# barrust/pyprobables

Measured on AMD Instinct MI355X. Metric: million keys/sec insert+lookup (Bloom m=2^28 k=7, CMS 2^20x5), higher is better.
Workload: dtype u64; 1 GPU; cfg2 Bloom m=2^28 k=7: per rank per step clear + insert 10M 16B keys + (merge) + check them; keys_per_rank=10000000, key_bytes=16, m_bits=268435456, k=7, parallelism=single GPU

## Files before the change

### pyprobables_amd/csrc/psk_part_bins.hpp

```cpp
#pragma once
#include "psk_partition.hpp"

namespace psk {

#ifndef PSK_BINS_NT
#define PSK_BINS_NT 768
#endif
constexpr int kBinThreads = PSK_BINS_NT;
constexpr int kBinMinWaves = kBinThreads <= 512 ? 4 : (kBinThreads <= 768 ? 6 : 8);
#ifndef PSK_BINS_KPT
#define PSK_BINS_KPT 2
#endif
constexpr int kBinKpt = PSK_BINS_KPT;
constexpr int kBinSlicesPerLane = 2;

template <class Pay>
struct pay_bins_ok { static constexpr bool value = false; };
template <>
struct pay_bins_ok<PayNone> { static constexpr bool value = true; };
template <>
struct pay_bins_ok<PayTileTag> { static constexpr bool value = true; };
template <>
struct pay_bins_ok<PayWeightSmall> { static constexpr bool value = true; };

constexpr uint32_t kBinHead = 2;
template <class Src, class IdxFn, class Pay, class Spill, int KT, int KPT>
__global__ __launch_bounds__(kBinThreads, kBinMinWaves) void k_part_bins(Src src, IdxFn idxfn, Pay pay, Spill spill, PartGeom g, uint32_t n, uint32_t cap,
                                                              uint32_t stride, uint32_t *segcnt, uint4 *buckets)
{
    constexpr int NT = kBinThreads;
    extern __shared__ __attribute__((aligned(16))) uint32_t smem[];
    char *lds = reinterpret_cast<char *>(smem);
    const uint32_t B = g.nbuckets;
    constexpr bool kExactK = KT != 8;
    const uint32_t k = kExactK ? (uint32_t)KT : g.k;
    const uint32_t mask = (1u << g.shift) - 1;
    const uint32_t tk = g.tile;
    const uint32_t ntiles = (n + tk - 1) / tk;
    const uint32_t last = n ? n - 1 : 0;
    const uint32_t stride4 = stride * 4u;
    const uint32_t lg_slices = 31u - (uint32_t)__builtin_clz(B);
    const uint32_t full4 = (cap + kBinHead) * 4u;
    constexpr uint32_t kCnt = 4;

    uint32_t L = 1;
    while (2 * L * B <= (uint32_t)NT) L *= 2;
    constexpr int kSlicesPerLane = kBinSlicesPerLane;
    const uint32_t sub = B <= (uint32_t)NT ? threadIdx.x % L : 0u;
    uint32_t myb[kSlicesPerLane], cur[kSlicesPerLane];
    uint4 *seg[kSlicesPerLane];
#pragma unroll
    for (int s = 0; s < kSlicesPerLane; ++s) {
        myb[s] = B <= (uint32_t)NT ? (s == 0 && threadIdx.x / L < B ? threadIdx.x / L : ~0u) : threadIdx.x + (uint32_t)s * NT;
        if (myb[s] >= B) myb[s] = ~0u;
        cur[s] = 0;
        seg[s] = buckets + (seg_index(g, 0, blockIdx.x) + (myb[s] == ~0u ? 0u : myb[s])) * g.segcap;
    }
    for (uint32_t b = threadIdx.x; b < B; b += NT) *reinterpret_cast<uint32_t *>(lds + b * stride4 + kCnt) = kBinHead * 4u;

    const uint32_t dbg = kBenchKnobs ? g.dbg : 0u;
    unsigned long long *t_acc = reinterpret_cast<unsigned long long *>(lds + (size_t)B * stride4 + 32);
    unsigned long long t_prev = 0;
    const bool t_lane = (dbg & 32) && (threadIdx.x == 0 || threadIdx.x == NT - 64);
    const uint32_t t_base = threadIdx.x == 0 ? 0u : 4u;
    if ((dbg & 32) && threadIdx.x < 8) t_acc[threadIdx.x] = 0;
#define PSK_BIN_TICK(ph)                                                 \
    if (t_lane) {                                                        \
        const unsigned long long t_now = __builtin_readcyclecounter();   \
        t_acc[t_base + (ph)] += t_now - t_prev;                          \
        t_prev = t_now;                                                  \
    }
    uint32_t fold = 0;
    constexpr bool WP = pay_weighted_plain<Pay>::value;
    typename Src::Key kcur[KPT];
    uint32_t wcur[WP ? KPT : 1];
    long long tally_s = 0;
    unsigned long long tally_a = 0;
    uint32_t tally_b = 0;
    {
        const uint32_t b0 = blockIdx.x * tk;
#pragma unroll
        for (int q = 0; q < KPT; ++q) {
            const uint32_t i = b0 + (uint32_t)q * NT + threadIdx.x;
            kcur[q] = src.load(i < last ? i : last);
            if constexpr (WP) wcur[q] = pay(i < last ? i : last, 0);
        }
    }
    lds_barrier();
    if (t_lane) t_prev = __builtin_readcyclecounter();

    uint32_t ordinal = ~0u;
    for (uint32_t tile = blockIdx.x; tile < ntiles; tile += gridDim.x) {
        ++ordinal;
        const uint32_t base = tile * tk;
        const uint32_t tile_end = base + tk < n ? base + tk : n;
        if constexpr (PSK_EXP_PRIO == 1) __builtin_amdgcn_s_setprio(0);
#pragma unroll
        for (int q = 0; q < KPT; ++q) {
            const uint32_t i = base + (uint32_t)q * NT + threadIdx.x;
            if ((uint32_t)q * NT < tk && i < tile_end) {
                uint32_t val[KT], bin[KT];
                uint32_t wfield = 0, wbig = 0, wq = 0;
                if constexpr (WP) {
                    wq = wcur[q];
                    if (pay.tally) {
                        const long long v = pay.weights_signed ? (long long)(int32_t)wq : (long long)wq;
                        tally_s += v;
                        tally_a += (unsigned long long)(v < 0 ? -v : v);
                        tally_b += (uint32_t)(wq >= (1u << kSmallWeightBits));
                    }
                    wbig = wq >= (1u << kSmallWeightBits) ? 1u : 0u;
                    wfield = wbig ? 0u : wq << 15;
                }
                if constexpr (IdxFn::lo32) {
                    uint32_t h[KT];
                    if (dbg & 4) {
#pragma unroll
                        for (int j = 0; j < KT; ++j) h[j] = (uint32_t)(((uint64_t)(i * 2654435761u + (uint32_t)j * 40503u) * 0x9E3779B97F4A7C15ULL) >> 13);
                    } else {
                        src.template hash32<KT>(kcur[q], i, 0u, h);
                    }
#pragma unroll
                    for (int j = 0; j < KT; ++j) {
                        if constexpr (std::is_same<IdxFn, IdxBloom<true>>::value || std::is_same<IdxFn, IdxBloomWide<true>>::value) {
                            val[j] = h[j] & mask;
                            bin[j] = __builtin_amdgcn_ubfe(h[j], g.shift, lg_slices);
                        } else {
                            const uint32_t x = idxfn.from32((uint32_t)j, h[j]);
                            val[j] = x & mask;
                            bin[j] = x >> g.shift;
                        }
                    }
                } else {
                    uint64_t h[KT];
                    src.template hash<KT>(kcur[q], i, 0u, h);
#pragma unroll
                    for (int j = 0; j < KT; ++j) {
                        const uint32_t x = idxfn((uint32_t)j, h[j]);
                        val[j] = x & mask;
                        bin[j] = x >> g.shift;
                    }
                }
                if (dbg & 2) {
#pragma unroll
                    for (int j = 0; j < KT; ++j) fold ^= val[j] + bin[j];
                    continue;
                }
                uint32_t at[KT], r4[KT], worst = 0;
#pragma unroll
                for (int j = 0; j < KT; ++j) {
                    r4[j] = 0;
                    if ((uint32_t)j < k) {
                        at[j] = __umul24(bin[j], stride4);
                        r4[j] = atomicAdd(reinterpret_cast<uint32_t *>(lds + at[j] + kCnt), 4u);
                    }
                }
#pragma unroll
                for (int j = 0; j < KT; ++j) {
                    if ((uint32_t)j < k) {
                        worst = r4[j] > worst ? r4[j] : worst;
                        *reinterpret_cast<uint32_t *>(lds + at[j] + (r4[j] < full4 ? r4[j] : full4)) = WP ? (val[j] | wfield) : val[j];
                    }
                }
                if constexpr (WP) {
                    if (wbig) {
#pragma unroll
                        for (int j = 0; j < KT; ++j)
                            if ((uint32_t)j < k) spill((bin[j] << g.shift) | val[j], wq);
                    }
                }
                if (worst >= full4) {
#pragma unroll
                    for (int j = 0; j < KT; ++j)
                        if ((uint32_t)j < k && r4[j] >= full4) {
                            if constexpr (pay_tile_tag<Pay>::value) spill((bin[j] << g.shift) | val[j], tile);
                            else if constexpr (WP) { if (!wbig) spill((bin[j] << g.shift) | val[j], wq); }
                            else spill((bin[j] << g.shift) | val[j], 0u);
                        }
                }
            }
        }
        {
            const uint32_t nb = (tile + gridDim.x) * tk;
#pragma unroll
            for (int q = 0; q < KPT; ++q) {
                const uint32_t i = nb + (uint32_t)q * NT + threadIdx.x;
                kcur[q] = src.load(i < last ? i : last);
                if constexpr (WP) wcur[q] = pay(i < last ? i : last, 0);
            }
        }
        if (dbg & 2) {
            if (fold == 0x12345u) segcnt[0] = fold;
            continue;
        }
        PSK_BIN_TICK(0);
        lds_barrier();
        PSK_BIN_TICK(1);
        if constexpr (PSK_EXP_PRIO == 1) __builtin_amdgcn_s_setprio(3);

        const uint32_t t0 = pay_tile_tag<Pay>::value ? (ordinal & 3u) << 2 : 0u, t1 = pay_tile_tag<Pay>::value ? ordinal & 12u : 0u;
#pragma unroll
        for (int s = 0; s < kSlicesPerLane; ++s) {
            const uint32_t b = myb[s];
            if (b == ~0u) continue;
            const char *bin = lds + b * stride4;
            const uint32_t c4 = *reinterpret_cast<const uint32_t *>(bin + kCnt);
            const uint32_t c = ((c4 < full4 ? c4 : full4) >> 2) - kBinHead;
            const uint32_t whole = c / 6u, rem = c - 6u * whole, ngroups = whole + (rem ? 1u : 0u);
            const uint2 *e = reinterpret_cast<const uint2 *>(bin + kBinHead * 4u);
            uint4 *out = seg[s] + cur[s];
            if (cur[s] + ngroups <= g.segcap) {
                const uint32_t hi0 = (3u | t0) << 28, hi1 = (3u | t1) << 28;
                for (uint32_t gq = sub; gq < whole; gq += L) {
                    const uint2 a0 = e[3 * gq], a1 = e[3 * gq + 1], a2 = e[3 * gq + 2];
                    uint4 o;
                    o.x = a0.x | (a0.y << 20);
                    o.y = (a0.y >> 12) | (a1.x << 8) | hi0;
                    o.z = a1.y | (a2.x << 20);
                    o.w = (a2.x >> 12) | (a2.y << 8) | hi1;
                    if (!(dbg & 1)) out[gq] = o;
                }
                if (rem && sub == (whole & (L - 1))) {
                    const uint2 a0 = e[3 * whole], a1 = e[3 * whole + 1], a2 = e[3 * whole + 2];
                    uint32_t f[6] = {a0.x, a0.y, a1.x, a1.y, a2.x, a2.y};
#pragma unroll
                    for (int x = 1; x < 6; ++x)
                        if ((uint32_t)x >= rem) f[x] = WP ? 0u : mask;
                    const uint32_t n0 = rem < 3u ? rem : 3u, n1 = rem - n0;
                    uint4 o;
                    o.x = f[0] | (f[1] << 20);
                    o.y = (f[1] >> 12) | (f[2] << 8) | ((n0 | t0) << 28);
                    o.z = f[3] | (f[4] << 20);
                    o.w = (f[4] >> 12) | (f[5] << 8) | ((n1 | t1) << 28);
                    if (!(dbg & 1)) out[whole] = o;
                }
            } else {
                for (uint32_t gq = sub; gq < ngroups; gq += L) {
                    const uint2 a0 = e[3 * gq], a1 = e[3 * gq + 1], a2 = e[3 * gq + 2];
                    uint32_t f[6] = {a0.x, a0.y, a1.x, a1.y, a2.x, a2.y};
                    const uint32_t left = c - 6u * gq, nv = left < 6u ? left : 6u;
#pragma unroll
                    for (int x = 1; x < 6; ++x)
                        if ((uint32_t)x >= nv) f[x] = WP ? 0u : mask;
                    const uint32_t n0 = nv < 3u ? nv : 3u, n1 = nv - n0;
                    if (cur[s] + gq < g.segcap) {
                        uint4 o;
                        o.x = f[0] | (f[1] << 20);
                        o.y = (f[1] >> 12) | (f[2] << 8) | ((n0 | t0) << 28);
                        o.z = f[3] | (f[4] << 20);
                        o.w = (f[4] >> 12) | (f[5] << 8) | ((n1 | t1) << 28);
                        out[gq] = o;
                    } else {
#pragma unroll
                        for (int x = 0; x < 6; ++x)
                            if ((uint32_t)x < nv) {
                                if constexpr (pay_tile_tag<Pay>::value) spill((b << g.shift) | f[x], tile);
                                else if constexpr (WP) spill((b << g.shift) | (f[x] & mask), f[x] >> 15);
                                else spill((b << g.shift) | f[x], 0u);
                            }
                    }
                }
            }
            cur[s] += ngroups;
        }
#pragma unroll
        for (int s = 0; s < kSlicesPerLane; ++s)
            if (myb[s] != ~0u && sub == 0) *reinterpret_cast<uint32_t *>(lds + myb[s] * stride4 + kCnt) = kBinHead * 4u;
#pragma unroll
        for (int q = 0; q < KPT; ++q) {
            Src::pin(kcur[q]);
            if constexpr (WP) asm volatile("" : "+v"(wcur[q]));
        }
        PSK_BIN_TICK(2);
        lds_barrier();
        PSK_BIN_TICK(3);
    }
    if (t_lane) {
        unsigned long long *prof = reinterpret_cast<unsigned long long *>(segcnt + (size_t)g.nbuckets * g.nwg);
        for (int ph = 0; ph < 4; ++ph) atomicAdd(prof + 1 + t_base + ph, t_acc[t_base + ph]);
        if (threadIdx.x == 0) atomicAdd(prof, 1ULL);
    }
#undef PSK_BIN_TICK
    if constexpr (WP) {
        if (pay.tally) {
            for (int o = 32; o > 0; o >>= 1) {
                tally_s += __shfl_down(tally_s, o);
                tally_a += __shfl_down(tally_a, o);
                tally_b += __shfl_down(tally_b, o);
            }
            unsigned long long *red = reinterpret_cast<unsigned long long *>(smem);
            if ((threadIdx.x & 63) == 0) {
                red[3 * (threadIdx.x >> 6)] = (unsigned long long)tally_s;
                red[3 * (threadIdx.x >> 6) + 1] = tally_a;
                red[3 * (threadIdx.x >> 6) + 2] = tally_b;
            }
            lds_barrier();
            if (threadIdx.x == 0) {
                unsigned long long ss = 0, aa = 0, bb = 0;
                for (int w = 0; w < NT / 64; ++w) { ss += red[3 * w]; aa += red[3 * w + 1]; bb += red[3 * w + 2]; }
                pay.tally[blockIdx.x] = make_ulonglong4(ss, aa, bb, 0ULL);
            }
        }
    }
#pragma unroll
    for (int s = 0; s < kSlicesPerLane; ++s)
        if (myb[s] != ~0u && sub == 0) segcnt[(uint64_t)myb[s] * g.nwg + blockIdx.x] = cur[s] < g.segcap ? cur[s] : g.segcap;
}

}
```

Before: 61580 Mkeys/s.

## Software-pipeline hashing of next tile's first key slot across bin write-out

Restructures the partition-bins kernel loop so the hash chain for slot 0 of the next tile is computed before the LDS barrier, while the current tile's bins are being written out. Key loads for the tile after that are issued as each slot is consumed, rather than all together at the end of the tile. The aim is to overlap ALU hashing and global loads with the LDS write-out phase and the barrier stalls. The cost is extra live registers for the precomputed hash values, so it is gated per template by a maximum KT, with the old loop kept as a fallback.

```diff
diff --git a/pyprobables_amd/csrc/psk_part_bins.hpp b/pyprobables_amd/csrc/psk_part_bins.hpp
--- a/pyprobables_amd/csrc/psk_part_bins.hpp
+++ b/pyprobables_amd/csrc/psk_part_bins.hpp
@@ -13,6 +13,16 @@
 #endif
 constexpr int kBinKpt = PSK_BINS_KPT;
 constexpr int kBinSlicesPerLane = 2;
+#ifndef PSK_BINS_PIPE
+#define PSK_BINS_PIPE 1
+#endif
+constexpr bool kBinPipe = PSK_BINS_PIPE != 0;
+template <class Src, class IdxFn, class Pay, int KT>
+struct bins_pipe {
+    static constexpr bool kWeighted = pay_weighted_plain<Pay>::value, kMulti = std::is_same<Src, KeysFixed16Multi>::value;
+    static constexpr int kMaxKt = IdxFn::lo32 ? (kWeighted ? 5 : (kMulti ? 7 : 8)) : (kWeighted ? 4 : 5);
+    static constexpr bool value = kBinPipe && KT <= kMaxKt;
+};
 
 template <class Pay>
 struct pay_bins_ok { static constexpr bool value = false; };
@@ -77,127 +87,93 @@
     long long tally_s = 0;
     unsigned long long tally_a = 0;
     uint32_t tally_b = 0;
-    {
-        const uint32_t b0 = blockIdx.x * tk;
-#pragma unroll
-        for (int q = 0; q < KPT; ++q) {
-            const uint32_t i = b0 + (uint32_t)q * NT + threadIdx.x;
-            kcur[q] = src.load(i < last ? i : last);
-            if constexpr (WP) wcur[q] = pay(i < last ? i : last, 0);
-        }
-    }
-    lds_barrier();
-    if (t_lane) t_prev = __builtin_readcyclecounter();
-
-    uint32_t ordinal = ~0u;
-    for (uint32_t tile = blockIdx.x; tile < ntiles; tile += gridDim.x) {
-        ++ordinal;
-        const uint32_t base = tile * tk;
-        const uint32_t tile_end = base + tk < n ? base + tk : n;
-        if constexpr (PSK_EXP_PRIO == 1) __builtin_amdgcn_s_setprio(0);
-#pragma unroll
-        for (int q = 0; q < KPT; ++q) {
-            const uint32_t i = base + (uint32_t)q * NT + threadIdx.x;
-            if ((uint32_t)q * NT < tk && i < tile_end) {
-                uint32_t val[KT], bin[KT];
-                uint32_t wfield = 0, wbig = 0, wq = 0;
-                if constexpr (WP) {
-                    wq = wcur[q];
-                    if (pay.tally) {
-                        const long long v = pay.weights_signed ? (long long)(int32_t)wq : (long long)wq;
-                        tally_s += v;
-                        tally_a += (unsigned long long)(v < 0 ? -v : v);
-                        tally_b += (uint32_t)(wq >= (1u << kSmallWeightBits));
-                    }
-                    wbig = wq >= (1u << kSmallWeightBits) ? 1u : 0u;
-                    wfield = wbig ? 0u : wq << 15;
-                }
-                if constexpr (IdxFn::lo32) {
-                    uint32_t h[KT];
-                    if (dbg & 4) {
-#pragma unroll
-                        for (int j = 0; j < KT; ++j) h[j] = (uint32_t)(((uint64_t)(i * 2654435761u + (uint32_t)j * 40503u) * 0x9E3779B97F4A7C15ULL) >> 13);
-                    } else {
-                        src.template hash32<KT>(kcur[q], i, 0u, h);
-                    }
-#pragma unroll
-                    for (int j = 0; j < KT; ++j) {
-                        if constexpr (std::is_same<IdxFn, IdxBloom<true>>::value || std::is_same<IdxFn, IdxBloomWide<true>>::value) {
-                            val[j] = h[j] & mask;
-                            bin[j] = __builtin_amdgcn_ubfe(h[j], g.shift, lg_slices);
-                        } else {
-                            const uint32_t x = idxfn.from32((uint32_t)j, h[j]);
-                            val[j] = x & mask;
-                            bin[j] = x >> g.shift;
-                        }
-                    }
-                } else {
-                    uint64_t h[KT];
-                    src.template hash<KT>(kcur[q], i, 0u, h);
-#pragma unroll
-                    for (int j = 0; j < KT; ++j) {
-                        const uint32_t x = idxfn((uint32_t)j, h[j]);
-                        val[j] = x & mask;
-                        bin[j] = x >> g.shift;
-                    }
-                }
-                if (dbg & 2) {
-#pragma unroll
-                    for (int j = 0; j < KT; ++j) fold ^= val[j] + bin[j];
-                    continue;
-                }
-                uint32_t at[KT], r4[KT], worst = 0;
-#pragma unroll
-                for (int j = 0; j < KT; ++j) {
-                    r4[j] = 0;
-                    if ((uint32_t)j < k) {
-                        at[j] = __umul24(bin[j], stride4);
-                        r4[j] = atomicAdd(reinterpret_cast<uint32_t *>(lds + at[j] + kCnt), 4u);
-                    }
-                }
-#pragma unroll
-                for (int j = 0; j < KT; ++j) {
-                    if ((uint32_t)j < k) {
-                        worst = r4[j] > worst ? r4[j] : worst;
-                        *reinterpret_cast<uint32_t *>(lds + at[j] + (r4[j] < full4 ? r4[j] : full4)) = WP ? (val[j] | wfield) : val[j];
-                    }
-                }
-                if constexpr (WP) {
-                    if (wbig) {
-#pragma unroll
-                        for (int j = 0; j < KT; ++j)
-                            if ((uint32_t)j < k) spill((bin[j] << g.shift) | val[j], wq);
-                    }
-                }
-                if (worst >= full4) {
-#pragma unroll
-                    for (int j = 0; j < KT; ++j)
-                        if ((uint32_t)j < k && r4[j] >= full4) {
-                            if constexpr (pay_tile_tag<Pay>::value) spill((bin[j] << g.shift) | val[j], tile);
-                            else if constexpr (WP) { if (!wbig) spill((bin[j] << g.shift) | val[j], wq); }
-                            else spill((bin[j] << g.shift) | val[j], 0u);
-                        }
-                }
-            }
-        }
-        {
-            const uint32_t nb = (tile + gridDim.x) * tk;
-#pragma unroll
-            for (int q = 0; q < KPT; ++q) {
-                const uint32_t i = nb + (uint32_t)q * NT + threadIdx.x;
-                kcur[q] = src.load(i < last ? i : last);
-                if constexpr (WP) wcur[q] = pay(i < last ? i : last, 0);
-            }
+    const uint32_t gstride = __builtin_amdgcn_readfirstlane(gridDim.x);
+
+    auto load_slot = [&](int q, uint32_t tb) {
+        const uint32_t i = tb + (uint32_t)q * NT + threadIdx.x;
+        kcur[q] = src.load(i < last ? i : last);
+        if constexpr (WP) wcur[q] = pay(i < last ? i : last, 0);
+    };
+    auto pin_slot = [&](int q) {
+        Src::pin(kcur[q]);
+        if constexpr (WP) asm volatile("" : "+v"(wcur[q]));
+    };
+    constexpr bool kHashIsIndex = IdxFn::lo32 && (std::is_same<IdxFn, IdxBloom<true>>::value || std::is_same<IdxFn, IdxBloomWide<true>>::value);
+    auto chains = [&](const typename Src::Key &key, uint32_t i, uint32_t (&x)[KT]) {
+        if constexpr (IdxFn::lo32) {
+            uint32_t h[KT];
+            if (dbg & 4) {
+#pragma unroll
+                for (int j = 0; j < KT; ++j) h[j] = (uint32_t)(((uint64_t)(i * 2654435761u + (uint32_t)j * 40503u) * 0x9E3779B97F4A7C15ULL) >> 13);
+            } else {
+                src.template hash32<KT>(key, i, 0u, h);
+            }
+#pragma unroll
+            for (int j = 0; j < KT; ++j) x[j] = kHashIsIndex ? h[j] : idxfn.from32((uint32_t)j, h[j]);
+        } else {
+            uint64_t h[KT];
+            src.template hash<KT>(key, i, 0u, h);
+#pragma unroll
+            for (int j = 0; j < KT; ++j) x[j] = idxfn((uint32_t)j, h[j]);
+        }
+    };
+    auto slots = [&](const uint32_t (&x)[KT], uint32_t wq, uint32_t tile) {
+        uint32_t val[KT], bin[KT];
+#pragma unroll
+        for (int j = 0; j < KT; ++j) {
+            val[j] = x[j] & mask;
+            bin[j] = kHashIsIndex ? __builtin_amdgcn_ubfe(x[j], g.shift, lg_slices) : x[j] >> g.shift;
         }
         if (dbg & 2) {
-            if (fold == 0x12345u) segcnt[0] = fold;
-            continue;
-        }
-        PSK_BIN_TICK(0);
-        lds_barrier();
-        PSK_BIN_TICK(1);
-        if constexpr (PSK_EXP_PRIO == 1) __builtin_amdgcn_s_setprio(3);
-
+#pragma unroll
+            for (int j = 0; j < KT; ++j) fold ^= val[j] + bin[j];
+            return;
+        }
+        uint32_t wfield = 0, wbig = 0;
+        if constexpr (WP) {
+            if (pay.tally) {
+                const long long v = pay.weights_signed ? (long long)(int32_t)wq : (long long)wq;
+                tally_s += v;
+                tally_a += (unsigned long long)(v < 0 ? -v : v);
+                tally_b += (uint32_t)(wq >= (1u << kSmallWeightBits));
+            }
+            wbig = wq >= (1u << kSmallWeightBits) ? 1u : 0u;
+            wfield = wbig ? 0u : wq << 15;
+        }
+        uint32_t at[KT], r4[KT], worst = 0;
+#pragma unroll
+        for (int j = 0; j < KT; ++j) {
+            r4[j] = 0;
+            if ((uint32_t)j < k) {
+                at[j] = __umul24(bin[j], stride4);
+                r4[j] = atomicAdd(reinterpret_cast<uint32_t *>(lds + at[j] + kCnt), 4u);
+            }
+        }
+#pragma unroll
+        for (int j = 0; j < KT; ++j) {
+            if ((uint32_t)j < k) {
+                worst = r4[j] > worst ? r4[j] : worst;
+                *reinterpret_cast<uint32_t *>(lds + at[j] + (r4[j] < full4 ? r4[j] : full4)) = WP ? (val[j] | wfield) : val[j];
+            }
+        }
+        if constexpr (WP) {
+            if (wbig) {
+#pragma unroll
+                for (int j = 0; j < KT; ++j)
+                    if ((uint32_t)j < k) spill((bin[j] << g.shift) | val[j], wq);
+            }
+        }
+        if (worst >= full4) {
+#pragma unroll
+            for (int j = 0; j < KT; ++j)
+                if ((uint32_t)j < k && r4[j] >= full4) {
+                    if constexpr (pay_tile_tag<Pay>::value) spill((bin[j] << g.shift) | val[j], tile);
+                    else if constexpr (WP) { if (!wbig) spill((bin[j] << g.shift) | val[j], wq); }
+                    else spill((bin[j] << g.shift) | val[j], 0u);
+                }
+        }
+    };
+    auto write_out = [&](uint32_t tile, uint32_t ordinal) {
         const uint32_t t0 = pay_tile_tag<Pay>::value ? (ordinal & 3u) << 2 : 0u, t1 = pay_tile_tag<Pay>::value ? ordinal & 12u : 0u;
 #pragma unroll
         for (int s = 0; s < kSlicesPerLane; ++s) {
@@ -266,14 +242,92 @@
 #pragma unroll
         for (int s = 0; s < kSlicesPerLane; ++s)
             if (myb[s] != ~0u && sub == 0) *reinterpret_cast<uint32_t *>(lds + myb[s] * stride4 + kCnt) = kBinHead * 4u;
-#pragma unroll
-        for (int q = 0; q < KPT; ++q) {
-            Src::pin(kcur[q]);
-            if constexpr (WP) asm volatile("" : "+v"(wcur[q]));
-        }
-        PSK_BIN_TICK(2);
+    };
+
+#pragma unroll
+    for (int q = 0; q < KPT; ++q) load_slot(q, blockIdx.x * tk);
+    uint32_t ordinal = ~0u;
+    if constexpr (bins_pipe<Src, IdxFn, Pay, KT>::value) {
+        uint32_t x0[KT], w0 = 0;
+#pragma unroll
+        for (int q = 0; q < KPT; ++q) pin_slot(q);
+        chains(kcur[0], blockIdx.x * tk + threadIdx.x, x0);
+        if constexpr (WP) w0 = wcur[0];
+        load_slot(0, (blockIdx.x + gstride) * tk);
         lds_barrier();
-        PSK_BIN_TICK(3);
+        if (t_lane) t_prev = __builtin_readcyclecounter();
+        for (uint32_t tile = blockIdx.x; tile < ntiles; tile += gstride) {
+            ++ordinal;
+            const uint32_t base = tile * tk, nb = base + gstride * tk;
+            const uint32_t tile_end = base + tk < n ? base + tk : n;
+            if constexpr (PSK_EXP_PRIO == 1) __builtin_amdgcn_s_setprio(0);
+            if (base + threadIdx.x < tile_end) slots(x0, w0, tile);
+#pragma unroll
+            for (int q = 1; q < KPT; ++q) {
+                const uint32_t i = base + (uint32_t)q * NT + threadIdx.x;
+                uint32_t x[KT];
+                if ((uint32_t)q * NT < tk && i < tile_end) chains(kcur[q], i, x);
+                const uint32_t wq = WP ? wcur[q] : 0u;
+                load_slot(q, nb);
+                if ((uint32_t)q * NT < tk && i < tile_end) slots(x, wq, tile);
+            }
+            if (!(dbg & 2)) {
+                PSK_BIN_TICK(0);
+                lds_barrier();
+            }
+#pragma unroll
+            for (int q = 0; q < KPT; ++q) pin_slot(q);
+            if (!(dbg & 2)) {
+                PSK_BIN_TICK(1);
+                if constexpr (PSK_EXP_PRIO == 1) __builtin_amdgcn_s_setprio(3);
+                write_out(tile, ordinal);
+                if constexpr (PSK_EXP_PRIO == 1) __builtin_amdgcn_s_setprio(0);
+                PSK_BIN_TICK(2);
+            }
+            chains(kcur[0], nb + threadIdx.x, x0);
+            if constexpr (WP) w0 = wcur[0];
+            load_slot(0, nb + gstride * tk);
+            if (dbg & 2) {
+                if (fold == 0x12345u) segcnt[0] = fold;
+                continue;
+            }
+            lds_barrier();
+            PSK_BIN_TICK(3);
+        }
+    } else {
+        lds_barrier();
+        if (t_lane) t_prev = __builtin_readcyclecounter();
+        for (uint32_t tile = blockIdx.x; tile < ntiles; tile += gridDim.x) {
+            ++ordinal;
+            const uint32_t base = tile * tk;
+            const uint32_t tile_end = base + tk < n ? base + tk : n;
+            if constexpr (PSK_EXP_PRIO == 1) __builtin_amdgcn_s_setprio(0);
+#pragma unroll
+            for (int q = 0; q < KPT; ++q) {
+                const uint32_t i = base + (uint32_t)q * NT + threadIdx.x;
+                if ((uint32_t)q * NT < tk && i < tile_end) {
+                    uint32_t x[KT];
+                    chains(kcur[q], i, x);
+                    slots(x, WP ? wcur[q] : 0u, tile);
+                }
+            }
+#pragma unroll
+            for (int q = 0; q < KPT; ++q) load_slot(q, (tile + gridDim.x) * tk);
+            if (dbg & 2) {
+                if (fold == 0x12345u) segcnt[0] = fold;
+                continue;
+            }
+            PSK_BIN_TICK(0);
+            lds_barrier();
+            PSK_BIN_TICK(1);
+            if constexpr (PSK_EXP_PRIO == 1) __builtin_amdgcn_s_setprio(3);
+            write_out(tile, ordinal);
+#pragma unroll
+            for (int q = 0; q < KPT; ++q) pin_slot(q);
+            PSK_BIN_TICK(2);
+            lds_barrier();
+            PSK_BIN_TICK(3);
+        }
     }
     if (t_lane) {
         unsigned long long *prof = reinterpret_cast<unsigned long long *>(segcnt + (size_t)g.nbuckets * g.nwg);
```

Result: faster. 64030 Mkeys/s (median of 6 runs) (+4.0%).
